# mct10/Speech-Vecalign

Hardware: AMD Instinct MI355X
Metric: aligned doc-pairs/sec (higher is better)
Workload: dtype bf16; 1 GPU; synthetic 4096x4096 d=1024 bf16 embeddings, 4 overlap layers/side, 10 alignment types, band 14, coarse-to-fine (max_size_full_dp=300), 1024 doc-pairs per GPU per step; pipeline=1, N=4096, M=4096, d=1024, overlaps=4, parallelism=dp1 (pairs sharded, no collective)

## Files before the change

speech-vecalign_amd/csrc/svx_api.hip:

```cpp
#include <stdarg.h>
#include <stdio.h>
#include <stdlib.h>
#include <string.h>

#include <chrono>
#include <functional>
#include <memory>
#include <type_traits>
#include <vector>

#include "svx_common.h"

static char g_err[512] = "";

int svx_fail(svx_ctx* ctx, int code, const char* fmt, ...) {
    char* dst = ctx ? ctx->err : g_err;
    va_list ap;
    va_start(ap, fmt);
    vsnprintf(dst, 512, fmt, ap);
    va_end(ap);
    return code;
}

static const char* kStageNames[] = {"pyr0",       "pyrN",     "pyr_aux",      "knob_scoresN", "knob",      "dense_costs",
                                    "dense_dp",   "path",     "band_costs0",  "band_costsN",  "band_dp0",  "band_dpN",
                                    "traceback",  "setup",    "total",        "host_plan",    "host_launch", "knob_sort", "knob_scores0", "pyr1", "tiles",
                                    "traceback0", "path0"};
enum {
    S_PYR0 = 0, S_PYRN, S_PYR_AUX, S_KNOB_SCORES, S_KNOB, S_DENSE_COSTS, S_DENSE_DP, S_PATH, S_BAND_COSTS0, S_BAND_COSTSN,
    S_BAND_DP0, S_BAND_DPN, S_TRACEBACK, S_SETUP, S_TOTAL, S_HOST_PLAN, S_HOST_LAUNCH, S_KNOB_SORT, S_KNOB_SCORES0, S_PYR1, S_TILES,
    S_TRACEBACK0, S_PATH0, S_COUNT
};

struct StageRec {
    int stage;
    hipEvent_t a, b;
};

struct BatchParams {
    SvxTypes tfinal, t11;
    int W, B, dtype, d, nsamp, n_types;
    double frac;
    bool straight, tiles, packable;
    bool around;
};

struct HalfState {
    char* arena = nullptr;
    size_t arena_bytes = 0;
    SvxPairDev* pinned = nullptr;
    size_t pinned_cap = 0;
    std::vector<SvxPairDev> host;
    SvxPairDev* dpairs = nullptr;
    int n_pairs = 0;
    int maxL = 0, max_ksum = 0, max_kn = 0, max_ds0 = 0, max_ds1 = 0, max_n0 = 0, max_tnd = 0;
    int max_nblk[SVX_MAX_LEVELS] = {0}, max_A[SVX_MAX_LEVELS] = {0};
    bool any_L0 = false;
    size_t o_tickets = 0;
    size_t o_planes = 0, b_planes = 0;
    double b_pyr[SVX_MAX_LEVELS] = {0}, b_bc[SVX_MAX_LEVELS] = {0}, b_knobN = 0, b_knob0 = 0, dense_cells = 0;
    BatchParams bp;
    bool chain_pending = false;
    bool chain_done_valid = false;
    hipEvent_t front_done = nullptr, chain_done = nullptr, upload_done = nullptr;
    bool upload_valid = false;
};

struct svx_ctx_ext : svx_ctx {
    double ms[S_COUNT];
    int launches[S_COUNT];
    std::vector<StageRec> recs;
    std::vector<StageRec> pending;
    double acc_ms[S_COUNT];
    long long acc_launches[S_COUNT];
    int pipeline;
    HalfState half[2];
    int last_split;
    hipStream_t chain;
    bool chain_ready;
    std::vector<hipEvent_t> ev_pool;
    size_t ev_next;
    hipStream_t side;
    hipStream_t helper;
    hipEvent_t side_fork, side_join;
// ... 766 lines not shown
        static const bool inline_sort = getenv("SVX_SORT_INLINE") != nullptr;
        if (parts > 1 && !inline_sort) SVX_HIP(ctx, hipStreamWaitEvent(cx->side, evs->pass[0][parts - 1], 0));
        ctx->stream = inline_sort ? main_stream : cx->side;
        int rc;
        {
            StageScope sc(ctx, S_KNOB_SORT);
            rc = svxl_knob_scores(ctx, h->dpairs, np, h->maxL, h->max_kn, h->max_n0, dtype, d, 0);
        }
        ctx->stream = main_stream;
        if (rc) return rc;
        SVX_HIP(ctx, hipEventRecord(cx->side_join, inline_sort ? main_stream : cx->side));
        return SVX_OK;
    };
    if (parts == 1) ops.push_back({0.0, -1, sort_op});
    for (int l = 0; l <= H.maxL; l++) {
        for (int q = 0; q < parts; q++) {
            const int lo = (int)((long long)np * q / parts), hi = (int)((long long)np * (q + 1) / parts);
            const double aux_us = (l == 0 ? 700.0 * waves : 250.0) / parts;
            if (parts == 1) {
                ops.push_back({aux_us, S_PYR_AUX, [=]() { return svxl_pyramid_level(ctx, h->dpairs, np, l, dtype, d, h->max_nblk[l], h->max_ksum, 0); }});
                ops.push_back({H.b_pyr[l] / (l == 0 ? 4.9e6 : 5.3e6), l == 0 ? S_PYR0 : (l == 1 ? S_PYR1 : S_PYRN),
                               [=]() { return svxl_pyramid_level(ctx, h->dpairs, np, l, dtype, d, h->max_nblk[l], h->max_ksum, 1); }});
                continue;
            }
            ops.push_back({H.b_pyr[l] / (l == 0 ? 4.9e6 : 5.3e6) / parts, l == 0 ? S_PYR0 : (l == 1 ? S_PYR1 : S_PYRN), [=]() -> int {
                hipStream_t main_stream = ctx->stream;
                int rc;
                if (l == 0 && q == 0) {
                    StageScope sc(ctx, S_PYR_AUX);
                    if ((rc = svxl_pyramid_level(ctx, h->dpairs + lo, hi - lo, l, dtype, d, h->max_nblk[l], h->max_ksum, 0))) return rc;
                } else {
                    if (l > 0) SVX_HIP(ctx, hipStreamWaitEvent(cx->helper, evs->pass[l - 1][q], 0));
                    ctx->stream = cx->helper;
                    {
                        StageScope sc(ctx, S_PYR_AUX);
                        rc = svxl_pyramid_level(ctx, h->dpairs + lo, hi - lo, l, dtype, d, h->max_nblk[l], h->max_ksum, 0);
                    }
                    ctx->stream = main_stream;
                    if (rc) return rc;
                    hipEvent_t aux_done;
                    if ((rc = next_event(ctx, &aux_done))) return rc;
                    SVX_HIP(ctx, hipEventRecord(aux_done, cx->helper));
                    SVX_HIP(ctx, hipStreamWaitEvent(main_stream, aux_done, 0));
                }
                if ((rc = svxl_pyramid_level(ctx, h->dpairs + lo, hi - lo, l, dtype, d, h->max_nblk[l], h->max_ksum, 1))) return rc;
                if ((rc = next_event(ctx, &evs->pass[l][q]))) return rc;
                SVX_HIP(ctx, hipEventRecord(evs->pass[l][q], main_stream));
                return SVX_OK;
            }});
        }
        if (parts > 1 && l == 0) ops.push_back({0.0, -1, sort_op});
    }
    if (!bp.straight) {
        ops.push_back({H.dense_cells * 2.7e-5, S_DENSE_COSTS, [=]() -> int {
            int rc = svxl_dense_costs_batch(ctx, h->dpairs, np, h->max_ds0, h->max_ds1, dtype, d);
            if (rc) return rc;
            return svxl_knob_from_dots(ctx, h->dpairs, np, h->max_kn);
        }});
    }
    if (H.maxL >= 1) {
        ops.push_back({H.b_knobN / 16.5e6, S_KNOB_SCORES, [=]() -> int {
            SVX_HIP(ctx, hipStreamWaitEvent(ctx->stream, cx->side_join, 0));
            return svxl_knob_scores(ctx, h->dpairs, np, h->maxL, h->max_kn, h->max_n0, dtype, d, 1);
        }});
    }
    ops.push_back({H.b_knob0 / 8.5e6, S_KNOB_SCORES0, [=]() -> int {
        SVX_HIP(ctx, hipStreamWaitEvent(ctx->stream, cx->side_join, 0));
        return svxl_knob_scores(ctx, h->dpairs, np, h->maxL, h->max_kn, h->max_n0, dtype, d, 2);
    }});
}

struct Seg {
    std::vector<Op> lb;
    bool has_s = false;
    Op s;
};

static void chain_segs(svx_ctx* ctx, HalfState& H, std::vector<Seg>& segs) {
    HalfState* h = &H;
    const BatchParams bp = H.bp;
    const int np = H.n_pairs, d = bp.d, dtype = bp.dtype, W = bp.W, B = bp.B;
    const double waves = (double)((np + 1023) / 1024);
    Seg cur;
    cur.lb.push_back({(np * (H.maxL + 1) * 0.21 < 300.0 ? 300.0 : np * (H.maxL + 1) * 0.21), S_KNOB,
                      [=]() { return svxl_del_penalty_batch(ctx, h->dpairs, np, h->maxL + 1, bp.frac); }});
    if (!bp.straight)
        cur.lb.push_back({(H.max_ds0 + H.max_ds1) * 1.7 * waves, S_DENSE_DP, [=]() { return svxl_dense_stage_batch(ctx, h->dpairs, np, h->max_ds0); }});
    const int first_depth = H.maxL > 0 ? H.maxL - 1 : 0;
    for (int depth = first_depth; depth >= 0; depth--) {
        const SvxTypes ty = depth == 0 ? bp.tfinal : bp.t11;
        int lim2 = 0, tamax2 = 0;
        const bool v2 = !bp.tiles && svxl_band2_limits(ty, W, depth, dtype, d, &lim2, &tamax2);
        const int maxA = H.max_A[depth];
        const int src_rows = (H.maxL > 0 && !H.any_L0) ? maxA / 2 + 8 : maxA;
        cur.lb.push_back({maxA * 0.08 * waves + 60.0, depth == 0 ? S_PATH0 : S_PATH, [=]() {
            return svxl_search_path_batch(ctx, h->dpairs, np, depth, maxA, src_rows, v2 ? lim2 : SVX_BC_ROWS - SVX_BC_TB,
                                          bp.tiles ? 0 : (v2 ? tamax2 : SVX_BC_TAMAX));
        }});
        cur.has_s = true;
        if (bp.tiles) {
            cur.s = {1.0e4, S_TILES, [=]() {
                int* tk = reinterpret_cast<int*>(h->arena + h->o_tickets);
                float* planes = h->b_planes ? reinterpret_cast<float*>(h->arena + h->o_planes) : nullptr;
                return svxl_band_tiles_batch(ctx, h->dpairs, np, ty, W, dtype, h->max_tnd, tk, tk + (size_t)h->max_tnd * np + 1, planes);
            }};
        } else {
            cur.s = {H.b_bc[depth] / 4.0e6, depth == 0 ? S_BAND_COSTS0 : S_BAND_COSTSN, [=]() {
                return v2 ? svxl_band_costs2_batch(ctx, h->dpairs, np, depth, maxA, ty, W, dtype, d)
                          : svxl_band_costs_batch(ctx, h->dpairs, np, depth, maxA, ty, W, dtype, d);
            }};
        }
        segs.push_back(cur);
        cur = Seg();
        if (!bp.tiles)
            cur.lb.push_back({maxA * (0.21 + 0.054 * (ty.n > 1 ? ty.n : 0)) * waves, depth == 0 ? S_BAND_DP0 : S_BAND_DPN,
                              [=]() { return svxl_sparse_dp_batch(ctx, h->dpairs, np, depth, ty, B); }});
        cur.lb.push_back({maxA * 0.27 * waves, depth == 0 ? S_TRACEBACK0 : S_TRACEBACK, [=]() { return svxl_sparse_traceback_batch(ctx, h->dpairs, np, depth, B, maxA, bp.packable ? 1 : 0); }});
    }
    segs.push_back(cur);
}

static int ensure_streams(svx_ctx* ctx) {
    svx_ctx_ext* cx = X(ctx);
    if (!cx->side_ready) {
        int prio_lo = 0, prio_hi = 0;
        SVX_HIP(ctx, hipDeviceGetStreamPriorityRange(&prio_lo, &prio_hi));
        SVX_HIP(ctx, hipStreamCreateWithPriority(&cx->side, hipStreamNonBlocking, prio_lo));
        SVX_HIP(ctx, hipStreamCreateWithPriority(&cx->helper, hipStreamNonBlocking, prio_hi));
        SVX_HIP(ctx, hipEventCreateWithFlags(&cx->side_fork, hipEventDisableTiming));
        SVX_HIP(ctx, hipEventCreateWithFlags(&cx->side_join, hipEventDisableTiming));
        cx->side_ready = true;
    }
    if (!cx->chain_ready) {
        int prio_lo = 0, prio_hi = 0;
        SVX_HIP(ctx, hipDeviceGetStreamPriorityRange(&prio_lo, &prio_hi));
        SVX_HIP(ctx, hipStreamCreateWithPriority(&cx->chain, hipStreamNonBlocking, prio_hi));
        cx->chain_ready = true;
    }
    for (int h = 0; h < 2; h++) {
        if (!cx->half[h].front_done) SVX_HIP(ctx, hipEventCreateWithFlags(&cx->half[h].front_done, hipEventDisableTiming));
// ... 212 lines not shown
```

speech-vecalign_amd/csrc/svx_common.h:

```cpp
#pragma once
#include <hip/hip_runtime.h>
#include <stdint.h>
#include <stddef.h>
#include "../../include/svx.h"

#define SVX_WAVE 64

#ifndef SVX_PYR_SLOTS
#define SVX_PYR_SLOTS 32
#endif
#define SVX_BC_TA 32
#define SVX_BC_TAMAX 64
#define SVX_BC_TB 16
#define SVX_BC_ROWS 48

struct ElemF32 {
    using storage = float;
    static constexpr int VEC = 4;
    static constexpr int DT = SVX_F32;
};
struct ElemF16 {
    using storage = uint16_t;
    static constexpr int VEC = 8;
    static constexpr int DT = SVX_F16;
// ... 193 lines not shown
    int8_t y[SVX_MAX_TYPES + 2];
};

struct svx_ctx {
    int device;
    hipStream_t stream;
    char* arena;
    size_t arena_bytes;
    size_t arena_used;
    char err[512];
    int profiling;
    char* post_buf;
    size_t post_bytes;
    char* post_pin[2];
    size_t post_pin_cap[2];
    hipEvent_t post_up[2];
    int post_up_valid[2];
    int post_turn;
};

int svx_fail(svx_ctx* ctx, int code, const char* fmt, ...);
#define NEED(ctx, cond, ...) \
    do { if (!(cond)) return svx_fail(ctx, SVX_ERR_ARG, __VA_ARGS__); } while (0)
inline bool aligned16(const void* p) { return (reinterpret_cast<uintptr_t>(p) & 15u) == 0; }
#define SVX_HIP(ctx, call)                                                                     \
    do {                                                                                       \
        hipError_t e_ = (call);                                                                \
        if (e_ != hipSuccess) return svx_fail(ctx, SVX_ERR_HIP, "%s: %s", #call, hipGetErrorString(e_)); \
    } while (0)
#define SVX_LAUNCH_CHECK(ctx, name)                                                            \
    do {                                                                                       \
        hipError_t e_ = hipGetLastError();                                                     \
        if (e_ != hipSuccess) return svx_fail(ctx, SVX_ERR_HIP, "launch %s: %s", name, hipGetErrorString(e_)); \
    } while (0)

int svxl_scratch_begin(svx_ctx*, const char* who, size_t up_bytes, size_t dev_bytes, char** pin, char** dev);
int svxl_scratch_upload(svx_ctx*, size_t bytes);
void svxl_scratch_release(svx_ctx*);
int svxl_make_norm1(svx_ctx*, float* vecs, int64_t rows, int d);
int svxl_pairsum(svx_ctx*, const float* vecs, int k, int n, int d, float* half, float* part, int nblk);
int svxl_colmean_plain(svx_ctx*, const float* part, int k, int nblk, int d, int count, float* mean);
int svxl_sub_mean(svx_ctx*, float* half, int k, int h, int d, const float* mean);
int svxl_sample_mean_plain(svx_ctx*, const float* vecs, int k, int n, int d, const int* idx, int S, float* rbar);
int svxl_norms_from_rbar(svx_ctx*, const float* vecs, int64_t rows, int d, const float* rbar, float* norms);
int svxl_gather_rows(svx_ctx*, const void* table, long long n_rows, int row_bytes, int dtype, const int* idx, long long n_out, void* out);
int svxl_pyramid_level(svx_ctx*, const SvxPairDev* pairs, int n_pairs, int level, int dtype, int d, int max_nblk,
                       int max_ksum, int part);
int svxl_score_path(svx_ctx*, const int* xx, const int* yy, int64_t n, const float* n1, const float* n2,
                    const float* v1, int rows1, const float* v2, int rows2, int d, float* out);
int svxl_knob_scores(svx_ctx*, const SvxPairDev* pairs, int n_pairs, int max_levels, int max_kn, int max_n0, int dtype, int d,
                     int part);
int svxl_dense_costs(svx_ctx*, const float* v0, int s0, const float* v1, int s1, int d, const float* n0,
                     const float* n1, int mul0, int mul1, float* costs);
int svxl_dense_costs_batch(svx_ctx*, const SvxPairDev* pairs, int n_pairs, int max_s0, int max_s1, int dtype, int d);
int svxl_knob_from_dots(svx_ctx*, const SvxPairDev* pairs, int n_pairs, int max_kn);
int svxl_band_costs(svx_ctx*, const void* v0, int k0, int n, const void* v1, int k1, int m, int d, int dtype,
                    const float* inv0, const float* inv1, const float* nrm0, const float* nrm1, const int* path,
                    int A, const SvxTypes& types, int W, float* costs, int* boff, int* status);
int svxl_band_costs_batch(svx_ctx*, const SvxPairDev* pairs, int n_pairs, int depth, int max_A, const SvxTypes& types,
                          int W, int dtype, int d);
bool svxl_band2_limits(const SvxTypes& types, int W, int depth, int dtype, int d, int* lim, int* tamax);
int svxl_band_costs2_batch(svx_ctx*, const SvxPairDev* pairs, int n_pairs, int depth, int max_A, const SvxTypes& types, int W,
                           int dtype, int d);
int svxl_band_tiles_shape(const SvxTypes& types);
size_t svxl_band_tiles_scratch(const SvxTypes& types);
int svxl_band_tiles_batch(svx_ctx*, const SvxPairDev* pairs, int n_pairs, const SvxTypes& types, int W, int dtype, int max_nd,
                          int* gpref, int* ticket, float* planes);
int svxl_dense_dp(svx_ctx*, const float* cost, int s0, int s1, float pen, double* csum, int* bp);
int svxl_dense_stage_batch(svx_ctx*, const SvxPairDev* pairs, int n_pairs, int max_s0);
int svxl_dense_traceback(svx_ctx*, const int* bp, int s0, int s1, int* align, int* count);
int svxl_sparse_dp(svx_ctx*, const float* costs, const int* boff_in, int A, int B, const SvxTypes& types, double pen,
                   int xs, int ys, double* csum, int* xp, int* yp, int* boff_out);
int svxl_sparse_dp_batch(svx_ctx*, const SvxPairDev* pairs, int n_pairs, int depth, const SvxTypes& types, int B);
int svxl_sparse_traceback(svx_ctx*, const double* csum, const int* xp, const int* yp, const int* boff, int a_out,
                          int B, int xs, int ys, int* align, double* scores, int* count);
int svxl_sparse_traceback_batch(svx_ctx*, const SvxPairDev* pairs, int n_pairs, int depth, int B, int max_A, int packed);
int svxl_search_path(svx_ctx*, const int* align, const int* n_align, int upsample, int size0, int size1, int* path,
                     int cap, int* path_len);
int svxl_search_path_batch(svx_ctx*, const SvxPairDev* pairs, int n_pairs, int depth, int max_rows, int max_src_rows, int chunk_lim,
                           int chunk_tamax);
int svxl_del_penalty(svx_ctx*, const float* scores, int64_t n, double frac, double* out);
int svxl_del_penalty_batch(svx_ctx*, const SvxPairDev* pairs, int n_pairs, int max_levels, double frac);
int svxl_prior_ingest_batch(svx_ctx*, const SvxPairDev* pairs, int n_pairs);
```

speech-vecalign_amd/csrc/svx_costs.hip:

```cpp
#include <stdlib.h>

#include "svx_common.h"

namespace {

typedef __attribute__((ext_vector_type(8))) __bf16 bf16x8_t;
typedef __attribute__((ext_vector_type(8))) _Float16 f16x8_t;
typedef __attribute__((ext_vector_type(4))) float f32x4_t;

constexpr int RS = 144;

template <typename E>
struct Mma;
template <>
struct Mma<ElemBF16> {
    static constexpr int KS = 64, NK = 2, KSTEP_BYTES = 64;
    using frag = uint4;
    __device__ static __forceinline__ int lane_off(int lane) { return (lane & 15) * RS + 16 * (lane >> 4); }
    __device__ static __forceinline__ frag load(const char* p) { return *reinterpret_cast<const uint4*>(p); }
    __device__ static __forceinline__ void mma(f32x4_t& acc, const frag& a, const frag& b) {
        acc = __builtin_amdgcn_mfma_f32_16x16x32_bf16(__builtin_bit_cast(bf16x8_t, a), __builtin_bit_cast(bf16x8_t, b), acc, 0, 0, 0);
    }
};
template <>
// ... 687 lines not shown
__global__ __launch_bounds__(BC_THREADS) void k_band_costs_batch(const SvxPairDev* __restrict__ pairs, int depth, SvxTypes ty,
                                                                 int kx, int ky, int W, int nchunk_b, int per_pair) {
    extern __shared__ __attribute__((aligned(16))) char smem[];
    const unsigned wg = xcd_remap(blockIdx.x, gridDim.x);
    const SvxPairDev& P = pairs[wg / per_pair];
    const int item = wg % per_pair;
    if (depth > P.L || (depth == P.L && P.L > 0)) return;
    const SvxLevel& Lv = P.lev[depth];
    BandArgs g;
    g.A = *Lv.path_len;
    const int chunk_a = item / nchunk_b;
    if (g.A <= 0 || chunk_a >= *Lv.nchunks) return;
    const int a0 = Lv.cstart[chunk_a], TAe = Lv.cstart[chunk_a + 1] - a0;
    g.n = Lv.n[0];
    g.m = Lv.n[1];
    g.d = P.d;
    g.v0 = LV0 ? P.v[0] : (const void*)Lv.P[0];
    g.v1 = LV0 ? P.v[1] : (const void*)Lv.P[1];
    g.inv0 = LV0 ? Lv.inv[0] : nullptr;
    g.inv1 = LV0 ? Lv.inv[1] : nullptr;
    g.nrm0 = Lv.nrm[0];
    g.nrm1 = Lv.nrm[1];
    g.path = Lv.path;
    g.W = W;
    g.costs = Lv.costs;
    g.boff = Lv.boff;
    g.status = P.status;
    g.atb = 1;
    band_block<E, NPT, SW>(g, ty, kx, ky, a0, TAe, item % nchunk_b, smem);
}

inline int nch_f32(int d) {
    int c = (d + 255) / 256;
    return c <= 1 ? 1 : c <= 2 ? 2 : c <= 4 ? 4 : 8;
}
inline int nch_16(int d) {
    int c = (d + 511) / 512;
    return c <= 1 ? 1 : c <= 2 ? 2 : 4;
}

constexpr size_t DENSE_SMEM = 2 * DT * sizeof(char*) + 2 * DT * RS;

}

int svxl_dense_costs(svx_ctx* ctx, const float* v0, int s0, const float* v1, int s1, int d, const float* n0,
                     const float* n1, int mul0, int mul1, float* costs) {
    if (s0 <= 0 || s1 <= 0) return SVX_OK;
    DenseArgs g{v0, v1, s0, s1, d, nullptr, nullptr, n0, n1, mul0, mul1, costs, nullptr};
    hipLaunchKernelGGL(k_dense_costs<ElemF32>, dim3((s0 + DT - 1) / DT, (s1 + DT - 1) / DT), dim3(256), DENSE_SMEM, ctx->stream, g);
    SVX_LAUNCH_CHECK(ctx, "k_dense_costs");
    return SVX_OK;
}

int svxl_dense_costs_batch(svx_ctx* ctx, const SvxPairDev* pairs, int n_pairs, int max_s0, int max_s1, int dtype, int d) {
    (void)d;
    if (n_pairs <= 0 || max_s0 <= 0 || max_s1 <= 0) return SVX_OK;
    dim3 grid((max_s0 + DT - 1) / DT, (max_s1 + DT - 1) / DT, n_pairs);
    hipLaunchKernelGGL((k_dense_costs_batch<ElemF32, false>), grid, dim3(256), DENSE_SMEM, ctx->stream, pairs);
    if (dtype == SVX_F32)
        hipLaunchKernelGGL((k_dense_costs_batch<ElemF32, true>), grid, dim3(256), DENSE_SMEM, ctx->stream, pairs);
    else if (dtype == SVX_F16)
        hipLaunchKernelGGL((k_dense_costs_batch<ElemF16, true>), grid, dim3(256), DENSE_SMEM, ctx->stream, pairs);
    else
        hipLaunchKernelGGL((k_dense_costs_batch<ElemBF16, true>), grid, dim3(256), DENSE_SMEM, ctx->stream, pairs);
    SVX_LAUNCH_CHECK(ctx, "k_dense_costs_batch");
    return SVX_OK;
}

int svxl_score_path(svx_ctx* ctx, const int* xx, const int* yy, int64_t n, const float* n1, const float* n2,
                    const float* v1, int rows1, const float* v2, int rows2, int d, float* out) {
    if (n <= 0) return SVX_OK;
    ScoreArgs g{v1, v2, nullptr, nullptr, n1, n2, xx, yy, n, rows1, rows2, d, out};
    int64_t nb = (n + 3) / 4;
    if (nb > 16384) nb = 16384;
#define M(N) hipLaunchKernelGGL((k_score_path<ElemF32, N>), dim3((unsigned)nb), dim3(256), 0, ctx->stream, g)
    switch (nch_f32(d)) {
        case 1: M(1); break;
        case 2: M(2); break;
        case 4: M(4); break;
        default: M(8); break;
    }
#undef M
    SVX_LAUNCH_CHECK(ctx, "k_score_path");
    return SVX_OK;
}

int svxl_knob_from_dots(svx_ctx* ctx, const SvxPairDev* pairs, int n_pairs, int max_kn) {
    if (n_pairs <= 0 || max_kn <= 0) return SVX_OK;
    int nb = (max_kn + 255) / 256;
    if (nb > 16) nb = 16;
    hipLaunchKernelGGL(k_knob_from_dots, dim3(nb, n_pairs), dim3(256), 0, ctx->stream, pairs);
    SVX_LAUNCH_CHECK(ctx, "k_knob_from_dots");
    return SVX_OK;
}

int svxl_knob_scores(svx_ctx* ctx, const SvxPairDev* pairs, int n_pairs, int max_L, int max_kn, int max_n0, int dtype, int d,
                     int part) {
    if (n_pairs <= 0 || max_kn <= 0) return SVX_OK;
    hipStream_t st = ctx->stream;
    const bool unsorted = (size_t)(max_n0 + 1) * sizeof(int) > 150 * 1024;
    if (unsorted) {
        if (part == 0) return SVX_OK;
        const int nbu = (max_kn + 3) / 4 < 2048 ? (max_kn + 3) / 4 : 2048;
#define U32(N, LV0, GY) hipLaunchKernelGGL((k_knob_scores_unsorted<ElemF32, N, LV0>), dim3(nbu, GY, n_pairs), dim3(256), 0, st, pairs)
#define U16(E, N) hipLaunchKernelGGL((k_knob_scores_unsorted<E, N, true>), dim3(nbu, 1, n_pairs), dim3(256), 0, st, pairs)
        if (part == 1) {
            if (max_L >= 1) {
                switch (nch_f32(d)) {
                    case 1: U32(1, false, max_L); break;
                    case 2: U32(2, false, max_L); break;
                    case 4: U32(4, false, max_L); break;
                    default: U32(8, false, max_L); break;
// ... 204 lines not shown
```

speech-vecalign_amd/csrc/svx_dp.hip:

```cpp
#include <stdlib.h>

#include "svx_common.h"

namespace {

struct DenseDpArgs {
    const float* cost;
    int s0, s1;
    float pen;
    double* csum;
    int* bp;
    int diag;
};

__device__ void dense_dp_block(const DenseDpArgs& g, double* ring) {
    const int rmax = g.s0 + 1, cmax = g.s1 + 1;
    const int tid = threadIdx.x, nt = blockDim.x;
    const double pen_d = (double)g.pen;
    auto cost_of = [&](int k, int r) -> float {
        const int c = k - r;
        return (r >= 1 && r <= g.s0 && c >= 1 && c <= g.s1) ? g.cost[(size_t)(r - 1) * g.s1 + (c - 1)] : 0.f;
    };
    float cnext = cost_of(0, tid);
    for (int k = 0; k <= g.s0 + g.s1; k++) {
        const int rlo = k - g.s1 > 0 ? k - g.s1 : 0;
        const int rhi = k < g.s0 ? k : g.s0;
        double* cur = ring + (size_t)(k % 3) * rmax;
        const double* p1 = ring + (size_t)((k + 2) % 3) * rmax;
        const double* p2 = ring + (size_t)((k + 1) % 3) * rmax;
        const float cfirst = cnext;
        {
            const int k1 = k + 1;
            const int rlo1 = k1 - g.s1 > 0 ? k1 - g.s1 : 0;
            cnext = cost_of(k1, rlo1 + tid);
        }
        for (int r = rlo + tid; r <= rhi; r += nt) {
            const int c = k - r;
            double v;
            int b;
            if (r == 0) {
                v = (double)((float)c * g.pen);
                b = 1;
                if (c == 0) { v = 0.0; b = 4; }
            } else if (c == 0) {
                v = (double)((float)r * g.pen);
                b = 2;
            } else {
                const float cf = (r == rlo + tid) ? cfirst : g.cost[(size_t)(r - 1) * g.s1 + (c - 1)];
                const double cost0 = p2[r - 1] + (double)cf;
                const double cost1 = p1[r] + pen_d;
                const double cost2 = p1[r - 1] + pen_d;
                v = cost0;
                b = 0;
                if (cost1 < v) { v = cost1; b = 1; }
                if (cost2 < v) { v = cost2; b = 2; }
            }
            cur[r] = v;
            g.bp[g.diag ? (size_t)k * rmax + r : (size_t)r * cmax + c] = b;
            if (g.csum) g.csum[(size_t)r * cmax + c] = v;
        }
        __syncthreads();
    }
}

__device__ int dense_traceback_thread(const int* bp, int s0, int s1, int* out, int diag = 0) {
    const int cmax = s1 + 1, rmax = s0 + 1;
    int xx = s0, yy = s1, n = 0;
    const int cap = s0 + s1;
    while (!(xx == 0 && yy == 0)) {
        if (n >= cap) return -SVX_ERR_BP;
        const int b = bp[diag ? (size_t)(xx + yy) * rmax + xx : (size_t)xx * cmax + yy];
        if ((xx == 0 && (b == 0 || b == 2)) || (yy == 0 && (b == 0 || b == 1))) return -SVX_ERR_BP;
        int* o = out + 4 * (size_t)(cap - 1 - n);
        if (b == 0) { o[0] = xx - 1; o[1] = 1; o[2] = yy - 1; o[3] = 1; xx--; yy--; }
        else if (b == 1) { o[0] = xx; o[1] = 0; o[2] = yy - 1; o[3] = 1; yy--; }
        else if (b == 2) { o[0] = xx - 1; o[1] = 1; o[2] = yy; o[3] = 0; xx--; }
        else return -SVX_ERR_BP;
        n++;
    }
    if (n < cap)
        for (int i = 0; i < n; i++)
            for (int c = 0; c < 4; c++) out[4 * (size_t)i + c] = out[4 * (size_t)(cap - n + i) + c];
    return n;
}

__global__ __launch_bounds__(256) void k_dense_dp(DenseDpArgs g) {
    extern __shared__ __attribute__((aligned(16))) char smem[];
    dense_dp_block(g, reinterpret_cast<double*>(smem));
}

__global__ void k_dense_traceback(const int* bp, int s0, int s1, int* align, int* count) {
    if (threadIdx.x == 0) *count = dense_traceback_thread(bp, s0, s1, align);
}

__global__ __launch_bounds__(256) void k_dense_stage_batch(const SvxPairDev* __restrict__ pairs) {
    extern __shared__ __attribute__((aligned(16))) char smem[];
    const SvxPairDev& P = pairs[blockIdx.x];
    if (*P.status != 0) return;
    const SvxLevel& Lv = P.lev[P.L];
    DenseDpArgs g;
    g.cost = P.dcost;
    g.s0 = Lv.n[0];
    g.s1 = Lv.n[1];
    g.pen = (float)(*Lv.pen);
    g.csum = nullptr;
    g.bp = P.dbp;
    g.diag = 1;
    dense_dp_block(g, reinterpret_cast<double*>(smem));
    if (threadIdx.x == 0) {
        const int n = dense_traceback_thread(P.dbp, g.s0, g.s1, Lv.align, 1);
        *Lv.n_align = n;
        if (n < 0) *P.status = -n;
    }
}

struct SparseDpArgs {
    const float* costs;
    const int* boff_in;
    int A, B;
    double pen;
    int xs, ys;
    double* csum;
    int* xp;
    int* yp;
    unsigned char* bpk;
    int* boff_out;
    int atb;
};

__device__ __forceinline__ size_t cost_index(const SparseDpArgs& g, int T, int t, int a, int b) {
    return g.atb ? ((size_t)a * T + t) * g.B + b : ((size_t)t * g.A + a) * g.B + b;
}
__device__ __forceinline__ void store_node(const SparseDpArgs& g, size_t o, double v, int bx, int by) {
    g.csum[o] = v;
    if (g.xp) { g.xp[o] = bx; g.yp[o] = by; }
    if (g.bpk) g.bpk[o] = bx < 0 ? (unsigned char)0xFF : (unsigned char)((bx << 4) | by);
}

constexpr int WIDE_CH = 32;
__host__ __device__ inline size_t wide_tab_bytes(int NTt) { return (size_t)WIDE_CH * (2 * NTt + 1) * sizeof(int) + (size_t)NTt * sizeof(int); }

template <bool RING>
__device__ void sparse_dp_block(const SparseDpArgs& g, const SvxTypes& ty, double* ring, int* tab) {
    const int tid = threadIdx.x, nt = blockDim.x;
    const int A = g.A, B = g.B, Aout = g.A + 2;
    const int T = ty.n, NTt = ty.n + 2;
    const int RD = ty.maxstep + 1;
    const int x_out = g.xs + 1, y_out = g.ys + 1;
    int* tpk = tab;
    int* shs = tab + NTt;
    int* sls = shs + WIDE_CH * NTt;
    int* bos = sls + WIDE_CH * NTt;
    for (int t = tid; t < NTt; t += nt) tpk[t] = (int)ty.x[t] | ((int)ty.y[t] << 8) | (((int)ty.x[t] + (int)ty.y[t]) << 16);
    for (int a = tid; a < Aout; a += nt) g.boff_out[a] = a < 2 ? g.boff_in[0] : g.boff_in[a - 2] + 1;
    __syncthreads();
    const double inf = __builtin_inf();
    for (int a0 = 0; a0 < Aout; a0 += WIDE_CH) {
        for (int e = tid; e < WIDE_CH * NTt; e += nt) {
            const int i = e / NTt, t = e - i * NTt;
            const int a = a0 + i, st = tpk[t] >> 16, yo = (tpk[t] >> 8) & 255;
            const int ap = a - st;
            int v = 1 << 24, sl = 0;
            if (a < Aout && ap >= 0) {
// ... 954 lines not shown
                ys[k] = 0.0 + (double)i / 1000.0 * res_max_d;
                k++;
            }
        }
        for (; k <= 27; k++) {
            xs[k] = (double)k * kstep;
            ys[k] = 0.0 + 1000.0 / 1000.0 * res_max_d;
        }
        xs[28] = 1.0;
        ys[28] = res_max_d;
        double res;
        if (frac < xs[0]) res = ys[0];
        else if (frac > xs[28]) res = ys[28];
        else {
            int j = 0;
            while (j < 28 && xs[j + 1] <= frac) j++;
            if (j == 28 || xs[j] == frac) res = ys[j];
            else {
                const double slope = (ys[j + 1] - ys[j]) / (xs[j + 1] - xs[j]);
                res = slope * (frac - xs[j]) + ys[j];
                if (res != res) {
                    res = slope * (frac - xs[j + 1]) + ys[j + 1];
                    if (res != res && ys[j] == ys[j + 1]) res = ys[j];
                }
            }
        }
        *out = res;
    }
}

__global__ __launch_bounds__(256) void k_del_penalty(const float* scores, long long n, double frac, double* out) {
    del_penalty_block(scores, n, frac, out);
}

__global__ __launch_bounds__(256) void k_del_penalty_batch(const SvxPairDev* __restrict__ pairs, double frac) {
    const SvxPairDev& P = pairs[blockIdx.y];
    const int level = blockIdx.x;
    if (level > P.L) return;
    const SvxLevel& Lv = P.lev[level];
    del_penalty_block(Lv.kscore, Lv.kn, frac, Lv.pen);
}

inline int dp_threads(int B) {
    int t = ((B + 63) / 64) * 64;
    return t < 64 ? 64 : (t > 1024 ? 1024 : t);
}

}

int svxl_dense_dp(svx_ctx* ctx, const float* cost, int s0, int s1, float pen, double* csum, int* bp) {
    const size_t smem = 3 * (size_t)(s0 + 1) * sizeof(double);
    if (smem > 150 * 1024) return svx_fail(ctx, SVX_ERR_ARG, "dense_dp: %d rows exceed the LDS ring (max 6399)", s0);
    DenseDpArgs g{cost, s0, s1, pen, csum, bp, 0};
    if (smem > 64 * 1024)
        SVX_HIP(ctx, hipFuncSetAttribute((const void*)k_dense_dp, hipFuncAttributeMaxDynamicSharedMemorySize, (int)smem));
    hipLaunchKernelGGL(k_dense_dp, dim3(1), dim3(256), smem, ctx->stream, g);
    SVX_LAUNCH_CHECK(ctx, "k_dense_dp");
    return SVX_OK;
}

int svxl_dense_stage_batch(svx_ctx* ctx, const SvxPairDev* pairs, int n_pairs, int max_s0) {
    if (n_pairs <= 0) return SVX_OK;
    const size_t smem = 3 * (size_t)(max_s0 + 1) * sizeof(double);
    if (smem > 150 * 1024) return svx_fail(ctx, SVX_ERR_ARG, "dense_dp: %d rows exceed the LDS ring (max 6399)", max_s0);
    if (smem > 64 * 1024)
        SVX_HIP(ctx, hipFuncSetAttribute((const void*)k_dense_stage_batch, hipFuncAttributeMaxDynamicSharedMemorySize, (int)smem));
    hipLaunchKernelGGL(k_dense_stage_batch, dim3(n_pairs), dim3(256), smem, ctx->stream, pairs);
    SVX_LAUNCH_CHECK(ctx, "k_dense_stage_batch");
    return SVX_OK;
}

int svxl_dense_traceback(svx_ctx* ctx, const int* bp, int s0, int s1, int* align, int* count) {
    hipLaunchKernelGGL(k_dense_traceback, dim3(1), dim3(64), 0, ctx->stream, bp, s0, s1, align, count);
    SVX_LAUNCH_CHECK(ctx, "k_dense_traceback");
    return SVX_OK;
}

static int dpf_groups(int T, int B) {
    int G = B <= 16 ? 4 : (B <= 32 ? 2 : 1);
    while (G > 1 && T < G) G >>= 1;
    return G;
}
static int dpf_tpl(int T, int B) {
    const int G = dpf_groups(T, B);
    int t = (T + G - 1) / G;
    if (t < 1) t = 1;
    return t <= 4 ? t : (t <= 6 ? 6 : 0);
}

static int dpf_choose_ch(int T, int B, int maxstep) {
    if (B > 64 || maxstep > 120) return 0;
    const int opts[8] = {64, 48, 32, 24, 16, 12, 8, 4};
    static const int budget_kb = [] { const char* e = getenv("SVX_DP_LDS_KB"); const int v = e ? atoi(e) : 36; return v >= 6 ? v : 36; }();
    for (int i = 0; i < 8; i++)
        if (dpf_smem_bytes(T, B, maxstep + 1, opts[i]) <= (size_t)budget_kb * 1024) return opts[i];
    for (int i = 0; i < 5; i++)
        if (dpf_smem_bytes(T, B, maxstep + 1, opts[i]) <= 52 * 1024) return opts[i];
    for (int i = 0; i < 8; i++)
        if (dpf_smem_bytes(T, B, maxstep + 1, opts[i]) <= 150 * 1024) return opts[i];
    return 0;
}

int svxl_sparse_dp(svx_ctx* ctx, const float* costs, const int* boff_in, int A, int B, const SvxTypes& types, double pen,
                   int xs, int ys, double* csum, int* xp, int* yp, int* boff_out) {
    if (A <= 0 || B <= 0) return SVX_OK;
    SparseDpArgs g{costs, boff_in, A, B, pen, xs, ys, csum, xp, yp, nullptr, boff_out, 0};
    const int CH = dpf_choose_ch(types.n, B, types.maxstep);
    if (CH > 0) {
        const size_t smem = dpf_smem_bytes(types.n, B, types.maxstep + 1, CH);
#define DPF_LAUNCH(TPLT, GG)                                                                                          \
    do {                                                                                                              \
        if (smem > 64 * 1024)                                                                                         \
            SVX_HIP(ctx, hipFuncSetAttribute((const void*)k_sparse_dp_fast<TPLT, GG>, hipFuncAttributeMaxDynamicSharedMemorySize, (int)smem)); \
        hipLaunchKernelGGL((k_sparse_dp_fast<TPLT, GG>), dim3(1), dim3(DPF_THREADS), smem, ctx->stream, g, types, CH); \
    } while (0)
#define DPF_LAUNCH_G(TPLT)                                                                                            \
    do {                                                                                                              \
        if (G == 4) DPF_LAUNCH(TPLT, 4); else if (G == 2) DPF_LAUNCH(TPLT, 2); else DPF_LAUNCH(TPLT, 1);               \
    } while (0)
        const int G = dpf_groups(types.n, B);
        switch (dpf_tpl(types.n, B)) {
// ... 159 lines not shown
```

Before: 9604 doc-pairs/s.

## Register-pipelined dense DP with LDS backpointer image and wave-parallel traceback

Replaces the dense anti-diagonal DP with a row-per-thread variant that prefetches cost values into registers several diagonals ahead. It also packs 2-bit backpointers into an LDS image so traceback reads LDS instead of global memory. The single-thread traceback becomes a wave-level walk whose outputs are flushed in coalesced 64-entry groups. Separately, the dense cost kernel launches are skipped when no pair needs the deep or L0 variant. The cost is more register pressure, extra LDS per block that may lower occupancy, and new stage counters.

Result: no change. 9593 doc-pairs/s (-0.1%).

```diff
diff --git a/speech-vecalign_amd/csrc/svx_api.hip b/speech-vecalign_amd/csrc/svx_api.hip
--- a/speech-vecalign_amd/csrc/svx_api.hip
+++ b/speech-vecalign_amd/csrc/svx_api.hip
@@ -25,11 +25,13 @@
 static const char* kStageNames[] = {"pyr0",       "pyrN",     "pyr_aux",      "knob_scoresN", "knob",      "dense_costs",
                                     "dense_dp",   "path",     "band_costs0",  "band_costsN",  "band_dp0",  "band_dpN",
                                     "traceback",  "setup",    "total",        "host_plan",    "host_launch", "knob_sort", "knob_scores0", "pyr1", "tiles",
-                                    "traceback0", "path0"};
+                                    "traceback0", "path0", "dense_walk_lds", "dense_walk_global"};
 enum {
     S_PYR0 = 0, S_PYRN, S_PYR_AUX, S_KNOB_SCORES, S_KNOB, S_DENSE_COSTS, S_DENSE_DP, S_PATH, S_BAND_COSTS0, S_BAND_COSTSN,
     S_BAND_DP0, S_BAND_DPN, S_TRACEBACK, S_SETUP, S_TOTAL, S_HOST_PLAN, S_HOST_LAUNCH, S_KNOB_SORT, S_KNOB_SCORES0, S_PYR1, S_TILES,
-    S_TRACEBACK0, S_PATH0, S_COUNT
+    S_TRACEBACK0, S_PATH0,
+    S_DENSE_WALK_LDS, S_DENSE_WALK_GLOBAL,
+    S_COUNT
 };
 
 struct StageRec {
@@ -902,8 +904,8 @@
         if (parts > 1 && l == 0) ops.push_back({0.0, -1, sort_op});
     }
     if (!bp.straight) {
-        ops.push_back({H.dense_cells * 2.7e-5, S_DENSE_COSTS, [=]() -> int {
-            int rc = svxl_dense_costs_batch(ctx, h->dpairs, np, h->max_ds0, h->max_ds1, dtype, d);
+        ops.push_back({H.dense_cells * 3.0e-5, S_DENSE_COSTS, [=]() -> int {
+            int rc = svxl_dense_costs_batch(ctx, h->dpairs, np, h->max_ds0, h->max_ds1, dtype, d, h->maxL >= 1, h->any_L0);
             if (rc) return rc;
             return svxl_knob_from_dots(ctx, h->dpairs, np, h->max_kn);
         }});
@@ -935,7 +937,12 @@
     cur.lb.push_back({(np * (H.maxL + 1) * 0.21 < 300.0 ? 300.0 : np * (H.maxL + 1) * 0.21), S_KNOB,
                       [=]() { return svxl_del_penalty_batch(ctx, h->dpairs, np, h->maxL + 1, bp.frac); }});
     if (!bp.straight)
-        cur.lb.push_back({(H.max_ds0 + H.max_ds1) * 1.7 * waves, S_DENSE_DP, [=]() { return svxl_dense_stage_batch(ctx, h->dpairs, np, h->max_ds0); }});
+        cur.lb.push_back({(H.max_ds0 + H.max_ds1) * 2.1 * waves, S_DENSE_DP, [=]() {
+            int lds = 0;
+            const int rc = svxl_dense_stage_batch(ctx, h->dpairs, np, h->max_ds0, h->max_ds1, &lds);
+            if (!rc) X(ctx)->launches[lds ? S_DENSE_WALK_LDS : S_DENSE_WALK_GLOBAL]++;
+            return rc;
+        }});
     const int first_depth = H.maxL > 0 ? H.maxL - 1 : 0;
     for (int depth = first_depth; depth >= 0; depth--) {
         const SvxTypes ty = depth == 0 ? bp.tfinal : bp.t11;
diff --git a/speech-vecalign_amd/csrc/svx_common.h b/speech-vecalign_amd/csrc/svx_common.h
--- a/speech-vecalign_amd/csrc/svx_common.h
+++ b/speech-vecalign_amd/csrc/svx_common.h
@@ -269,7 +269,8 @@
                      int part);
 int svxl_dense_costs(svx_ctx*, const float* v0, int s0, const float* v1, int s1, int d, const float* n0,
                      const float* n1, int mul0, int mul1, float* costs);
-int svxl_dense_costs_batch(svx_ctx*, const SvxPairDev* pairs, int n_pairs, int max_s0, int max_s1, int dtype, int d);
+int svxl_dense_costs_batch(svx_ctx*, const SvxPairDev* pairs, int n_pairs, int max_s0, int max_s1, int dtype, int d,
+                           bool any_deep, bool any_l0);
 int svxl_knob_from_dots(svx_ctx*, const SvxPairDev* pairs, int n_pairs, int max_kn);
 int svxl_band_costs(svx_ctx*, const void* v0, int k0, int n, const void* v1, int k1, int m, int d, int dtype,
                     const float* inv0, const float* inv1, const float* nrm0, const float* nrm1, const int* path,
@@ -284,7 +285,7 @@
 int svxl_band_tiles_batch(svx_ctx*, const SvxPairDev* pairs, int n_pairs, const SvxTypes& types, int W, int dtype, int max_nd,
                           int* gpref, int* ticket, float* planes);
 int svxl_dense_dp(svx_ctx*, const float* cost, int s0, int s1, float pen, double* csum, int* bp);
-int svxl_dense_stage_batch(svx_ctx*, const SvxPairDev* pairs, int n_pairs, int max_s0);
+int svxl_dense_stage_batch(svx_ctx*, const SvxPairDev* pairs, int n_pairs, int max_s0, int max_s1, int* lds_walk);
 int svxl_dense_traceback(svx_ctx*, const int* bp, int s0, int s1, int* align, int* count);
 int svxl_sparse_dp(svx_ctx*, const float* costs, const int* boff_in, int A, int B, const SvxTypes& types, double pen,
                    int xs, int ys, double* csum, int* xp, int* yp, int* boff_out);
diff --git a/speech-vecalign_amd/csrc/svx_costs.hip b/speech-vecalign_amd/csrc/svx_costs.hip
--- a/speech-vecalign_amd/csrc/svx_costs.hip
+++ b/speech-vecalign_amd/csrc/svx_costs.hip
@@ -763,12 +763,15 @@
     return SVX_OK;
 }
 
-int svxl_dense_costs_batch(svx_ctx* ctx, const SvxPairDev* pairs, int n_pairs, int max_s0, int max_s1, int dtype, int d) {
+int svxl_dense_costs_batch(svx_ctx* ctx, const SvxPairDev* pairs, int n_pairs, int max_s0, int max_s1, int dtype, int d,
+                           bool any_deep, bool any_l0) {
     (void)d;
     if (n_pairs <= 0 || max_s0 <= 0 || max_s1 <= 0) return SVX_OK;
     dim3 grid((max_s0 + DT - 1) / DT, (max_s1 + DT - 1) / DT, n_pairs);
-    hipLaunchKernelGGL((k_dense_costs_batch<ElemF32, false>), grid, dim3(256), DENSE_SMEM, ctx->stream, pairs);
-    if (dtype == SVX_F32)
+    if (any_deep)
+        hipLaunchKernelGGL((k_dense_costs_batch<ElemF32, false>), grid, dim3(256), DENSE_SMEM, ctx->stream, pairs);
+    if (!any_l0) {
+    } else if (dtype == SVX_F32)
         hipLaunchKernelGGL((k_dense_costs_batch<ElemF32, true>), grid, dim3(256), DENSE_SMEM, ctx->stream, pairs);
     else if (dtype == SVX_F16)
         hipLaunchKernelGGL((k_dense_costs_batch<ElemF16, true>), grid, dim3(256), DENSE_SMEM, ctx->stream, pairs);
diff --git a/speech-vecalign_amd/csrc/svx_dp.hip b/speech-vecalign_amd/csrc/svx_dp.hip
--- a/speech-vecalign_amd/csrc/svx_dp.hip
+++ b/speech-vecalign_amd/csrc/svx_dp.hip
@@ -63,37 +63,187 @@
     }
 }
 
-__device__ int dense_traceback_thread(const int* bp, int s0, int s1, int* out, int diag = 0) {
+#ifndef SVX_DENSE_D
+#define SVX_DENSE_D 16
+#endif
+constexpr int DENSE_D = SVX_DENSE_D;
+constexpr int DENSE_NT = 256;
+constexpr int DENSE_ROWS_MAX = 2 * DENSE_NT;
+
+__host__ __device__ inline int dense_img_pitch(int s1) { return (s1 + 1 + 15) / 16; }
+__host__ __device__ inline size_t dense_ring_bytes(int s0) { return 3 * (size_t)(s0 + 1) * sizeof(double); }
+__host__ __device__ inline size_t dense_img_bytes(int s0, int s1) { return (size_t)(s0 + 1) * dense_img_pitch(s1) * sizeof(unsigned); }
+
+template <int NJ>
+__device__ void dense_dp_rows(const DenseDpArgs& g, double* ring, unsigned* img) {
+    const int s0 = g.s0, s1 = g.s1;
+    const int rmax = s0 + 1, cmax = s1 + 1;
+    const int tid = threadIdx.x;
+    const double pen_d = (double)g.pen;
+    const int pitch = dense_img_pitch(s1);
+    int row[NJ];
+    size_t cbase[NJ];
+    float cr[NJ][DENSE_D];
+    double own[NJ], up1[NJ];
+    unsigned acc[NJ];
+#pragma unroll
+    for (int j = 0; j < NJ; j++) {
+        row[j] = 1 + tid + DENSE_NT * j;
+        const int rc = row[j] <= s0 ? row[j] : s0;
+        cbase[j] = (size_t)(rc - 1) * s1;
+        own[j] = 0.0;
+        up1[j] = 0.0;
+        acc[j] = 0u;
+    }
+    auto fetch = [&](int j, int k) -> float {
+        int c = k - row[j] - 1;
+        c = c < 0 ? 0 : (c > s1 - 1 ? s1 - 1 : c);
+        return gld(g.cost + cbase[j] + c);
+    };
+#pragma unroll
+    for (int i = 0; i < DENSE_D; i++)
+#pragma unroll
+        for (int j = 0; j < NJ; j++) cr[j][i] = fetch(j, i);
+    if (img)
+        for (int w = tid; w < pitch; w += DENSE_NT) img[w] = 0x55555555u;
+    const int nsteps = ((s0 + s1 + 1 + DENSE_D - 1) / DENSE_D) * DENSE_D;
+    for (int k0 = 0; k0 < nsteps; k0 += DENSE_D) {
+#pragma unroll
+        for (int i = 0; i < DENSE_D; i++) {
+            const int k = k0 + i;
+            double* cur = ring + (size_t)(k % 3) * rmax;
+            const double* p1 = ring + (size_t)((k + 2) % 3) * rmax;
+            if (tid == 0 && k <= s1) {
+                const double v = k == 0 ? 0.0 : (double)((float)k * g.pen);
+                cur[0] = v;
+                gst(g.bp + (g.diag ? (size_t)k * rmax : (size_t)k), k == 0 ? 4 : 1);
+                if (g.csum) gst(g.csum + k, v);
+            }
+#pragma unroll
+            for (int j = 0; j < NJ; j++) {
+                const int r = row[j];
+                const int c = k - r;
+                const float cf = cr[j][i];
+                cr[j][i] = fetch(j, k + DENSE_D);
+                if (r <= s0 && c >= 0 && c <= s1) {
+                    const double nb = p1[r - 1];
+                    double v;
+                    int b;
+                    if (c == 0) {
+                        v = (double)((float)r * g.pen);
+                        b = 2;
+                    } else {
+                        const double cost0 = up1[j] + (double)cf;
+                        const double cost1 = own[j] + pen_d;
+                        const double cost2 = nb + pen_d;
+                        v = cost0;
+                        b = 0;
+                        if (cost1 < v) { v = cost1; b = 1; }
+                        if (cost2 < v) { v = cost2; b = 2; }
+                    }
+                    own[j] = v;
+                    up1[j] = nb;
+                    cur[r] = v;
+                    gst(g.bp + (g.diag ? (size_t)k * rmax + r : (size_t)r * cmax + c), b);
+                    if (g.csum) gst(g.csum + (size_t)r * cmax + c, v);
+                    if (img) {
+                        acc[j] |= (unsigned)b << (2 * (c & 15));
+                        if ((c & 15) == 15 || c == s1) {
+                            img[(size_t)r * pitch + (c >> 4)] = acc[j];
+                            acc[j] = 0u;
+                        }
+                    }
+                }
+            }
+            __syncthreads();
+        }
+    }
+}
+
+__device__ int dense_traceback_block(const unsigned* img, const int* bp, int diag, int s0, int s1, int* out) {
+    __shared__ int sh_dn;
     const int cmax = s1 + 1, rmax = s0 + 1;
-    int xx = s0, yy = s1, n = 0;
     const int cap = s0 + s1;
-    while (!(xx == 0 && yy == 0)) {
-        if (n >= cap) return -SVX_ERR_BP;
-        const int b = bp[diag ? (size_t)(xx + yy) * rmax + xx : (size_t)xx * cmax + yy];
-        if ((xx == 0 && (b == 0 || b == 2)) || (yy == 0 && (b == 0 || b == 1))) return -SVX_ERR_BP;
-        int* o = out + 4 * (size_t)(cap - 1 - n);
-        if (b == 0) { o[0] = xx - 1; o[1] = 1; o[2] = yy - 1; o[3] = 1; xx--; yy--; }
-        else if (b == 1) { o[0] = xx; o[1] = 0; o[2] = yy - 1; o[3] = 1; yy--; }
-        else if (b == 2) { o[0] = xx - 1; o[1] = 1; o[2] = yy; o[3] = 0; xx--; }
-        else return -SVX_ERR_BP;
-        n++;
-    }
-    if (n < cap)
-        for (int i = 0; i < n; i++)
-            for (int c = 0; c < 4; c++) out[4 * (size_t)i + c] = out[4 * (size_t)(cap - n + i) + c];
+    const int pitch = dense_img_pitch(s1);
+    const bool al16 = (reinterpret_cast<size_t>(out) & 15) == 0;
+    if (__builtin_amdgcn_readfirstlane((int)(threadIdx.x >> 6)) == 0) {
+        int xx = __builtin_amdgcn_readfirstlane(s0), yy = __builtin_amdgcn_readfirstlane(s1), n = 0, err = 0;
+        int r0 = 0, r1 = 0, r2 = 0, r3 = 0;
+        int first_pending = 0;
+        auto flush = [&](int first, int last) {
+            const int idx = (first & ~63) + (int)threadIdx.x;
+            if (idx >= first && idx < last) {
+                int* o = out + 4 * (size_t)(cap - 1 - idx);
+                if (al16) gst16(o, (uint32_t)r0, (uint32_t)r1, (uint32_t)r2, (uint32_t)r3);
+                else { gst(o, r0); gst(o + 1, r1); gst(o + 2, r2); gst(o + 3, r3); }
+            }
+        };
+        for (;;) {
+            xx = __builtin_amdgcn_readfirstlane(xx);
+            yy = __builtin_amdgcn_readfirstlane(yy);
+            n = __builtin_amdgcn_readfirstlane(n);
+            if (xx == 0 && yy == 0) break;
+            if (n >= cap) { err = SVX_ERR_BP; break; }
+            int b;
+            if (img) b = (int)((img[(size_t)xx * pitch + (yy >> 4)] >> (2 * (yy & 15))) & 3u);
+            else b = gld(bp + (diag ? (size_t)(xx + yy) * rmax + xx : (size_t)xx * cmax + yy));
+            b = __builtin_amdgcn_readfirstlane(b);
+            if ((xx == 0 && (b == 0 || b == 2)) || (yy == 0 && (b == 0 || b == 1))) { err = SVX_ERR_BP; break; }
+            if (b < 0 || b > 2) { err = SVX_ERR_BP; break; }
+            const int dx = b != 1, dy = b != 2;
+            {
+                const bool me = (int)threadIdx.x == (n & 63);
+                r0 = me ? xx - dx : r0;
+                r1 = me ? dx : r1;
+                r2 = me ? yy - dy : r2;
+                r3 = me ? dy : r3;
+            }
+            xx -= dx;
+            yy -= dy;
+            n++;
+            if ((n & 63) == 0) {
+                flush(first_pending, n);
+                first_pending = n;
+            }
+        }
+        n = __builtin_amdgcn_readfirstlane(n);
+        if (first_pending < n) flush(first_pending, n);
+        if (threadIdx.x == 0) sh_dn = err ? -err : n;
+    }
+    __syncthreads();
+    const int n = sh_dn;
+    if (n < 0 || n >= cap) return n;
+    const int nt = blockDim.x;
+    for (int base = 0; base < n; base += nt) {
+        const int j = base + threadIdx.x;
+        int m0 = 0, m1 = 0, m2 = 0, m3 = 0;
+        if (j < n) {
+            const int* s = out + 4 * (size_t)(cap - n + j);
+            m0 = gld(s); m1 = gld(s + 1); m2 = gld(s + 2); m3 = gld(s + 3);
+        }
+        __syncthreads();
+        if (j < n) {
+            int* w = out + 4 * (size_t)j;
+            gst(w, m0); gst(w + 1, m1); gst(w + 2, m2); gst(w + 3, m3);
+        }
+        __syncthreads();
+    }
     return n;
 }
 
-__global__ __launch_bounds__(256) void k_dense_dp(DenseDpArgs g) {
+__global__ __launch_bounds__(DENSE_NT) void k_dense_dp(DenseDpArgs g, int mode) {
     extern __shared__ __attribute__((aligned(16))) char smem[];
-    dense_dp_block(g, reinterpret_cast<double*>(smem));
-}
-
-__global__ void k_dense_traceback(const int* bp, int s0, int s1, int* align, int* count) {
-    if (threadIdx.x == 0) *count = dense_traceback_thread(bp, s0, s1, align);
-}
-
-__global__ __launch_bounds__(256) void k_dense_stage_batch(const SvxPairDev* __restrict__ pairs) {
+    if (mode == 1) dense_dp_rows<1>(g, reinterpret_cast<double*>(smem), nullptr);
+    else if (mode == 2) dense_dp_rows<2>(g, reinterpret_cast<double*>(smem), nullptr);
+    else dense_dp_block(g, reinterpret_cast<double*>(smem));
+}
+
+__global__ __launch_bounds__(64) void k_dense_traceback(const int* bp, int s0, int s1, int* align, int* count) {
+    const int n = dense_traceback_block(nullptr, bp, 0, s0, s1, align);
+    if (threadIdx.x == 0) *count = n;
+}
+
+__global__ __launch_bounds__(DENSE_NT) void k_dense_stage_batch(const SvxPairDev* __restrict__ pairs, int lds_walk) {
     extern __shared__ __attribute__((aligned(16))) char smem[];
     const SvxPairDev& P = pairs[blockIdx.x];
     if (*P.status != 0) return;
@@ -106,9 +256,14 @@
     g.csum = nullptr;
     g.bp = P.dbp;
     g.diag = 1;
-    dense_dp_block(g, reinterpret_cast<double*>(smem));
+    double* ring = reinterpret_cast<double*>(smem);
+    const bool rows = g.s0 >= 1 && g.s1 >= 1 && g.s0 <= DENSE_ROWS_MAX;
+    unsigned* img = (rows && lds_walk) ? reinterpret_cast<unsigned*>(smem + ((dense_ring_bytes(g.s0) + 15) & ~(size_t)15)) : nullptr;
+    if (rows && g.s0 <= DENSE_NT) dense_dp_rows<1>(g, ring, img);
+    else if (rows) dense_dp_rows<2>(g, ring, img);
+    else dense_dp_block(g, ring);
+    const int n = dense_traceback_block(img, P.dbp, 1, g.s0, g.s1, Lv.align);
     if (threadIdx.x == 0) {
-        const int n = dense_traceback_thread(P.dbp, g.s0, g.s1, Lv.align, 1);
         *Lv.n_align = n;
         if (n < 0) *P.status = -n;
     }
@@ -1169,21 +1324,32 @@
     const size_t smem = 3 * (size_t)(s0 + 1) * sizeof(double);
     if (smem > 150 * 1024) return svx_fail(ctx, SVX_ERR_ARG, "dense_dp: %d rows exceed the LDS ring (max 6399)", s0);
     DenseDpArgs g{cost, s0, s1, pen, csum, bp, 0};
+    const int mode = (s0 >= 1 && s1 >= 1 && s0 <= DENSE_ROWS_MAX) ? (s0 <= DENSE_NT ? 1 : 2) : 0;
     if (smem > 64 * 1024)
         SVX_HIP(ctx, hipFuncSetAttribute((const void*)k_dense_dp, hipFuncAttributeMaxDynamicSharedMemorySize, (int)smem));
-    hipLaunchKernelGGL(k_dense_dp, dim3(1), dim3(256), smem, ctx->stream, g);
+    hipLaunchKernelGGL(k_dense_dp, dim3(1), dim3(DENSE_NT), smem, ctx->stream, g, mode);
     SVX_LAUNCH_CHECK(ctx, "k_dense_dp");
     return SVX_OK;
 }
 
-int svxl_dense_stage_batch(svx_ctx* ctx, const SvxPairDev* pairs, int n_pairs, int max_s0) {
+#ifndef SVX_DENSE_LDS_KB
+#define SVX_DENSE_LDS_KB 40
+#endif
+constexpr size_t DENSE_LDS_BUDGET = (size_t)SVX_DENSE_LDS_KB * 1024;
+
+int svxl_dense_stage_batch(svx_ctx* ctx, const SvxPairDev* pairs, int n_pairs, int max_s0, int max_s1, int* lds_walk) {
+    if (lds_walk) *lds_walk = 0;
     if (n_pairs <= 0) return SVX_OK;
-    const size_t smem = 3 * (size_t)(max_s0 + 1) * sizeof(double);
+    size_t smem = dense_ring_bytes(max_s0);
     if (smem > 150 * 1024) return svx_fail(ctx, SVX_ERR_ARG, "dense_dp: %d rows exceed the LDS ring (max 6399)", max_s0);
+    const size_t with_img = ((smem + 15) & ~(size_t)15) + dense_img_bytes(max_s0, max_s1);
+    const int lds = (max_s0 >= 1 && max_s1 >= 1 && max_s0 <= DENSE_ROWS_MAX && with_img <= DENSE_LDS_BUDGET) ? 1 : 0;
+    if (lds) smem = with_img;
     if (smem > 64 * 1024)
         SVX_HIP(ctx, hipFuncSetAttribute((const void*)k_dense_stage_batch, hipFuncAttributeMaxDynamicSharedMemorySize, (int)smem));
-    hipLaunchKernelGGL(k_dense_stage_batch, dim3(n_pairs), dim3(256), smem, ctx->stream, pairs);
+    hipLaunchKernelGGL(k_dense_stage_batch, dim3(n_pairs), dim3(DENSE_NT), smem, ctx->stream, pairs, lds);
     SVX_LAUNCH_CHECK(ctx, "k_dense_stage_batch");
+    if (lds_walk) *lds_walk = lds;
     return SVX_OK;
 }
 
```
